# meteofrance/py4cast

Hardware: AMD Instinct MI355X
Metric: AR-training samples/sec (512x512x60 grid, 3-step rollout) (higher is better)
Workload: dtype bf16; 1 GPU; HalfUNet scaled_ar rollout T=3, grid 512x512x60 (+5 forcings, 4 statics), WeightedLoss(MSE), AdamW, B=2/GPU; global_batch=2, parallelism=dp1, border_size=0, setup_steps=2, accumulate_grad_batches=1, hip_graph=False, deterministic_library_solvers=False, full=False

## Files before the change

include/py4cast_hip.h:

```cpp
#ifndef PY4CAST_HIP_H
#define PY4CAST_HIP_H

#include <stddef.h>
#include <stdint.h>

#ifdef __cplusplus
extern "C" {
#endif

#define P4C_VERSION 100

typedef void* p4c_stream_t;

enum p4c_error {
    P4C_OK = 0,
    P4C_ERR_INVALID = -1,
    P4C_ERR_LAUNCH = -2,
    P4C_ERR_RUNTIME = -3,
    P4C_ERR_UNSUPPORTED = -4
};

enum p4c_dtype { P4C_F32 = 0, P4C_BF16 = 1 };

enum p4c_loss_kind { P4C_LOSS_MSE = 0, P4C_LOSS_L1 = 1 };
// ... 140 lines not shown
                 int B, int H, int W, int m_blocks, p4c_stream_t stream);

size_t p4c_conv_wgrad_workspace_bytes(int CI_pad, int ks);
int p4c_conv_stat_tiles(int compute, int storage, int CI, int B, int H, int W);
int p4c_conv_stat_tiles_ks(int compute, int storage, int CI, int ks, int B, int H, int W);
int p4c_conv_kernel_kind(int compute, int storage, int CI, int ks, int B, int H, int W);
int p4c_conv_wgrad(const void* in, int compute, int storage, int CI_pad, int ks, const float* in_scale, const float* in_shift,
                   int in_relu, const void* dout, int CO, int CI, float* grad, void* workspace, int B, int H, int W,
                   p4c_stream_t stream);
int p4c_conv_wgrad_nb(const void* in, const float* in_scale, const float* in_shift, int in_relu, const void* dA, const void* y,
                      const float* gamma, const float* nscale, const float* nshift, const float* rstd, const float* mean,
                      const float* k1, const float* k2, int CO, int CI, float* grad, void* workspace, int B, int H, int W,
                      p4c_stream_t stream);
int p4c_upsample_sum_bwd_x(int storage, const void* dS, int B, int H, int W, void* tx1, void* tx2, void* tx3, void* tx4,
                           p4c_stream_t stream);

int p4c_out_conv_bwd_slots(int B, int64_t N);
size_t p4c_out_conv_bwd_workspace_bytes(int B, int64_t N);
int p4c_out_conv_bwd(const void* dy, const void* wprep_dgrad, const void* y, const float* scale, const float* shift, const float* mean,
                     const float* rstd, void* dA, float* stat_partial, int CO, float* grad_w, void* workspace, int B, int64_t N,
                     p4c_stream_t stream);
int p4c_conv_wgrad_kernel_kind(int storage, int B, int H, int W);
int p4c_conv_compact_supported(int in_c, int out_c, int ks, int B, int H, int W);
int p4c_conv_fwd_compact(const void* in, int in_c, const void* wprep, int ks, void* out, int out_c, int B, int H, int W,
                         p4c_stream_t stream);
int p4c_conv_wgrad_compact(const void* in, int in_c, int ks, const void* dout, int dout_c, int CO, int CI, float* grad, void* workspace,
                           int B, int H, int W, p4c_stream_t stream);

typedef struct p4c_halfunet_desc {
    int32_t B, H, W;
    int32_t cin;
    int32_t cin_pad;
    int32_t cout;
    int32_t dx_channels;
    int32_t dtype;
    int32_t norm;
    int32_t groups;
    int32_t has_bias;
    float eps;
    float momentum;
    int32_t compute;
    int32_t weights_prepared;
    int32_t skip_out_conv;
} p4c_halfunet_desc;

int p4c_first_conv_tail_slots(int B, int H, int W);
int p4c_first_conv_tail(const void* x, int x_cs, int cin, const float* w, void* y, float* stat_partial, int B, int H, int W, p4c_stream_t stream);

int p4c_set_side_stream(p4c_stream_t side, void* const* events, int n_events);
int p4c_side_stream_defer(int on);
int p4c_side_stream_enable(int on);
long long p4c_side_stream_launch_count(void);
int p4c_side_stream_join(p4c_stream_t stream);
int p4c_graph_replace_memsets(void* graph, int* replaced, int* left);

int64_t p4c_halfunet_param_count(const p4c_halfunet_desc* d);
int p4c_halfunet_workspace_bytes(const p4c_halfunet_desc* d, size_t* saved_bytes, size_t* scratch_bytes);
int p4c_halfunet_prepare_weights(const p4c_halfunet_desc* d, const float* params, void* scratch, p4c_stream_t stream);
int p4c_halfunet_forward(const p4c_halfunet_desc* d, const void* x, const float* params, float* running, void* y,
                         void* saved, void* scratch, int training, p4c_stream_t stream);
int p4c_halfunet_tail(const p4c_halfunet_desc* d, const float* params, void* saved, const void** a, const float** a_scale,
                      const float** a_shift, const float** wout);
int p4c_halfunet_backward(const p4c_halfunet_desc* d, const void* x, const float* params, const void* dy, void* dx,
                          float* grads, void* saved, void* scratch, int training, p4c_stream_t stream);


enum p4c_activation { P4C_ACT_NONE = 0, P4C_ACT_RELU = 1, P4C_ACT_SILU = 2 };

int p4c_edge_gather_add_fwd(const void* base, const void* a, const int32_t* ia, const void* b, const int32_t* ib,
                            void* out, int64_t E, int C, int dtype, int act, p4c_stream_t stream);
int p4c_edge_gather_add_bwd(const void* dh, const void* base, const void* a, const int32_t* ia, const void* b,
                            const int32_t* ib, void* dpre, int64_t E, int C, int dtype, int act, p4c_stream_t stream);
int p4c_segment_sum(const void* msg, const int32_t* offsets, const int32_t* perm, const void* init, void* out,
                    int64_t N, int64_t E, int C, int dtype, int out_dtype, p4c_stream_t stream);
int p4c_segment_sum_pair(const void* msg, const int32_t* offsets_a, const int32_t* perm_a, void* out_a, int64_t Na,
                         const int32_t* offsets_b, const int32_t* perm_b, void* out_b, int64_t Nb, int64_t E, int C, int dtype,
                         p4c_stream_t stream);


int p4c_window_attn_fwd(const void* qkv, const float* bias_t, void* out, int B, int Hp, int Wp, int heads, int head_dim,
                        int ws, int shift, float scale, int dtype, p4c_stream_t stream);
size_t p4c_window_attn_bwd_workspace_bytes(int B, int Hp, int Wp, int heads, int ws);
int p4c_window_attn_bwd(const void* qkv, const float* bias_t, const void* dout, void* dqkv, float* dbias_t, void* workspace,
                        int B, int Hp, int Wp, int heads, int head_dim, int ws, int shift, float scale, int dtype,
                        p4c_stream_t stream);


int p4c_row_layernorm_fwd(const void* x, const void* res, const float* gamma, const float* beta, float eps, void* out,
                          int64_t R, int C, int dtype, p4c_stream_t stream);
size_t p4c_row_layernorm_bwd_workspace_bytes(int64_t R, int C, int dtype);
int p4c_row_layernorm_bwd(const void* dy, const void* x, const float* gamma, float eps, void* dx, float* dgamma, float* dbeta,
                          void* workspace, int64_t R, int C, int dtype, p4c_stream_t stream);
int p4c_row_layernorm_fwd_masked(const void* x, const void* res, const float* gamma, const float* beta, float eps, void* out, int64_t R,
                                 int C, int dtype, int Hp, int Wp, int H, int W, p4c_stream_t stream);
int p4c_row_layernorm_bwd_masked(const void* dy, const void* x, const float* gamma, float eps, void* dx, float* dgamma, float* dbeta,
                                 void* workspace, int64_t R, int C, int dtype, int Hp, int Wp, int H, int W, p4c_stream_t stream);
int p4c_row_add_layernorm_fwd(const void* x, const void* add, int64_t add_rows, const float* gamma, const float* beta, float eps,
                              void* sum_out, void* out, int64_t R, int C, int dtype, p4c_stream_t stream);
size_t p4c_row_add_layernorm_bwd_workspace_bytes(int64_t R, int C);
int p4c_row_add_layernorm_bwd(const void* dy, const void* t, const void* extra, const float* gamma, float eps, void* dt, float* dgamma,
                              float* dbeta, void* workspace, int64_t R, int C, int dtype, p4c_stream_t stream);
int p4c_sum_leading(const void* x, int dtype, int nb, int64_t n, float* out, int accumulate, p4c_stream_t stream);
size_t p4c_row_linear_wgrad_workspace_bytes(int64_t R, int K);
int p4c_row_linear_wgrad(const void* dy, const void* x, float* dw_db, void* workspace, int64_t R, int O, int K, int dtype,
                         p4c_stream_t stream);

// ... 197 lines not shown
```

py4cast_amd/_lib_model.py:

```python

import ctypes
from ctypes import c_float, c_int, c_int32, c_int64, c_size_t, c_void_p

P, I, L, F = c_void_p, c_int, c_int64, c_float


class HalfUNetDesc(ctypes.Structure):

    _fields_ = [
        ("B", c_int32), ("H", c_int32), ("W", c_int32),
        ("cin", c_int32), ("cin_pad", c_int32), ("cout", c_int32), ("dx_channels", c_int32),
        ("dtype", c_int32), ("norm", c_int32), ("groups", c_int32), ("has_bias", c_int32),
        ("eps", c_float), ("momentum", c_float), ("compute", c_int32),
        ("weights_prepared", c_int32), ("skip_out_conv", c_int32),
    ]


DP = ctypes.POINTER(HalfUNetDesc)


class RowMlpDesc(ctypes.Structure):

    _fields_ = [
        ("rows", c_int64), ("x", c_void_p), ("k", c_int32), ("k_real", c_int32), ("w1", c_void_p), ("ldw1", c_int32),
# ... 68 lines not shown
    "p4c_gemm_nt": [P, L, P, I, I, I, I, I, I, I, I, P, P, L, I, P, P, L, P, L, P, P, P],
    "p4c_gemm_tn": [P, L, P, L, I, I, I, I, I, I, I, P, P, I, I, P, P],
    "p4c_bnorm_finalize": [P, I, ctypes.c_double, I, P, P, F, F, P, P, P, P, P, P, P, P],
    "p4c_upconv_prep_weight": [P, I, I, P, P, P],
    "p4c_gemm_upconv_fwd": [P, L, P, P, I, I, I, I, I, P, L, P, P],
    "p4c_gemm_upconv_dgrad": [P, L, P, I, I, I, I, I, P, L, P, P],
    "p4c_gemm_upconv_wgrad": [P, L, P, L, I, I, I, I, I, P, P, I, P, P],
    "p4c_unet_enc_tail_fwd": [P, P, P, P, L, P, I, I, I, I, I, P],
    "p4c_unet_enc_tail_bwd": [P, P, L, P, L, P, P, P, P, P, I, I, I, I, I, P],
    "p4c_seg_patch_gather": [P, P, I, I, I, I, I, I, I, P],
    "p4c_seg_patch_scatter": [P, P, I, I, I, I, I, I, I, I, P],
    "p4c_seg_chan_ln_fwd": [P, P, P, F, P, P, L, I, P],
    "p4c_seg_chan_ln_bwd": [P, P, P, P, F, P, P, P, L, I, P],
    "p4c_seg_reduce_partials": [P, I, I, P, I, P, I, P],
    "p4c_seg_dw3x3_fwd": [P, P, P, P, I, I, I, I, P],
    "p4c_seg_dw3x3_dgrad": [P, P, P, I, I, I, I, P],
    "p4c_seg_dw3x3_wgrad": [P, P, P, I, I, I, I, P],
    "p4c_seg_sra_fwd": [P, P, P, P, I, I, I, I, F, P],
    "p4c_seg_sra_bwd": [P, P, P, P, P, P, P, P, I, I, I, I, F, P],
    "p4c_seg_upsum_fwd": [P, P, P, P, P, I, I, I, I, P],
    "p4c_seg_upsum_bwd": [P, P, P, P, I, I, I, I, P],
    "p4c_upsample_bilinear_ac_fwd": [P, P, I, I, I, I, I, P],
    "p4c_upsample_bilinear_ac_bwd": [P, P, I, I, I, I, I, P],
    "p4c_deeplab_stem_fwd": [P, P, P, P, P, I, I, I, I, P],
    "p4c_deeplab_stem_bwd": [P, P, P, P, P, P, P, P, P, I, I, I, I, P],
    "p4c_deeplab_colsum": [P, L, P, I, I, I, I, P],
    "p4c_deeplab_pool_head_fwd": [P, I, I, P, P, P, F, F, P, P, P, I, I, I, I, P, P, P, P, P],
    "p4c_deeplab_pool_head_bwd": [P, I, P, P, P, P, P, P, I, I, I, I, P, P, P, P, P, P],
    "p4c_deeplab_pool_broadcast": [P, P, I, I, I, P],
    "p4c_deeplab_assemble_fwd": [P, P, P, P, P, P, I, I, I, P],
    "p4c_deeplab_assemble_bwd": [P, P, P, P, P, I, I, I, P],
}
OTHER = {
    "p4c_conv_wgrad_workspace_bytes": ([I, I], c_size_t),
    "p4c_out_conv_bwd_slots": ([I, L], c_int),
    "p4c_first_conv_tail_slots": ([I, I, I], c_int),
    "p4c_out_conv_bwd_workspace_bytes": ([I, L], c_size_t),
    "p4c_conv_stat_tiles": ([I, I, I, I, I, I], c_int),
    "p4c_conv_stat_tiles_ks": ([I, I, I, I, I, I, I], c_int),
    "p4c_conv_kernel_kind": ([I, I, I, I, I, I, I], c_int),
    "p4c_conv_compact_supported": ([I, I, I, I, I, I], c_int),
    "p4c_halfunet_param_count": ([DP], c_int64),
    "p4c_window_attn_bwd_workspace_bytes": ([I, I, I, I, I], c_size_t),
    "p4c_row_layernorm_bwd_workspace_bytes": ([L, I, I], c_size_t),
    "p4c_row_linear_wgrad_workspace_bytes": ([L, I], c_size_t),
    "p4c_row_gemm_supported": ([I, I], c_int),
    "p4c_row_gemm_wgrad_supported": ([I, I, I], c_int),
    "p4c_row_gemm_wgrad_workspace_bytes": ([L, I, I, I], c_size_t),
    "p4c_row_mlp_bwd_workspace_bytes": ([L, I], c_size_t),
    "p4c_row_mlp_prepared_bytes": ([I], c_size_t),
    "p4c_node_proj_wgrad_workspace_bytes": ([L, I], c_size_t),
    "p4c_grad_reduce_pending": ([], c_int),
    "p4c_side_stream_launch_count": ([], ctypes.c_longlong),
    "p4c_row_add_layernorm_bwd_workspace_bytes": ([L, I], c_size_t),
    "p4c_gemm_nt_workspace_bytes": ([I, I, I], c_size_t),
    "p4c_gemm_nt_stat_blocks": ([I, I, I], c_int),
    "p4c_gemm_tn_workspace_bytes": ([I, I, I], c_size_t),
    "p4c_unet_enc_tail_bwd_blocks": ([I, I, I, I], c_int),
    "p4c_seg_chan_ln_bwd_blocks": ([L], c_int),
    "p4c_seg_dw3x3_wgrad_rows": ([I, I, I], c_int),
    "p4c_seg_sra_bwd_workspace_bytes": ([I, I, I, I], c_size_t),
    "p4c_deeplab_stem_bwd_blocks": ([I, I, I, I], c_int),
}
```

py4cast_amd/csrc/halfunet.cpp:

```cpp
#include <stdlib.h>

#include <atomic>
#include <functional>
#include <vector>

#include "kernels.hpp"

namespace p4c {
namespace {

constexpr int NF = 64;
constexpr int NLEV = 5;
constexpr int NCONV = 12;
constexpr int NWSLOT = 2 * NCONV + 3;

struct Layout {
    int esz;
    int64_t n[NLEV];
    int Hk[NLEV], Wk[NLEV];
    int64_t w[NCONV], gamma[NCONV], beta[NCONV], wout, nparams;
    int64_t Y[NCONV], P[NLEV], S, act_elems, norm_base, norm[NCONV], saved_bytes;
    int64_t wslot_floats;
    int64_t wprep, statp, wgradp[NCONV + 1], ocbp[2], nbwdp, k1i[2][NCONV], k2i[2][NCONV], tickets, f_floats, g_base, G0, G1, G2, TB, DY[2][NCONV], scratch_bytes;
    int G;
};

inline int conv_level(int i) { return i < 10 ? i / 2 : 0; }
inline int conv_cin(const p4c_halfunet_desc& d, int i) { return i == 0 ? d.cin : NF; }
inline int conv_cin_pad(const p4c_halfunet_desc& d, int i) { return i == 0 ? d.cin_pad : NF; }
inline int64_t align256(int64_t v) { return (v + 255) / 256 * 256; }
inline int dx_blocks(const p4c_halfunet_desc& d) { return d.dx_channels > 64 ? (d.dx_channels + 63) / 64 : 1; }

inline int stat_tiles(int compute, int storage, int CI, int B, int H, int W, int ks = 3) {
    if (compute == P4C_BF16) return conv_bf16_stat_slots(CI, storage, B, H, W, ks);
    return ((H + CONV_TH - 1) / CONV_TH) * ((W + CONV_TW - 1) / CONV_TW);
}

inline int prep_w(int compute, const float* w, int CO, int CI, int ks, int tf, int M_pad, int K_pad, void* out, hipStream_t st) {
    return compute == P4C_BF16 ? prep_weights_bf16(w, CO, CI, ks, tf, M_pad, K_pad, out, st)
                               : prep_weights(w, CO, CI, ks, tf, M_pad, K_pad, (float*)out, st);
}
inline int conv_fwd(int compute, int storage, const void* in, int CI, const void* wp, int ks, const float* sc, const float* sh,
                    int relu, void* out, int out_cs, float* statp, int B, int H, int W, int mblocks, hipStream_t st,
                    const BatchFin* fin = nullptr, const RingBwdStats* bst = nullptr, int* nblk_out = nullptr,
                    const NormBwdCoef* nb = nullptr) {
    return compute == P4C_BF16
               ? conv_fwd_bf16(in, storage, CI, wp, ks, sc, sh, relu, out, out_cs, statp, B, H, W, mblocks, st, fin, bst, nblk_out, nb)
               : conv_fwd_f32((const float*)in, CI, (const float*)wp, ks, sc, sh, relu, nullptr, (float*)out, out_cs, statp, B, H, W,
                              mblocks, st);
}
inline int conv_wgrad(int compute, int storage, const void* in, int CI, int ks, const float* sc, const float* sh, int relu,
                      const void* dout, float* partial, int G, int B, int H, int W, int CO, int CIreal, float* grad,
                      hipStream_t st, const NormBwdCoef* nb = nullptr) {
    return compute == P4C_BF16
               ? conv_wgrad_bf16(in, storage, CI, ks, sc, sh, relu, dout, partial, G, B, H, W, CO, CIreal, grad, st, nb)
               : conv_wgrad_f32((const float*)in, CI, ks, sc, sh, relu, (const float*)dout, partial, G, B, H, W, CO, CIreal, grad, st);
}

int check_desc(const p4c_halfunet_desc* d) {
    P4C_CHECK_ARG(d, "halfunet: null descriptor");
    P4C_CHECK_ARG(d->B > 0 && d->H > 0 && d->W > 0, "halfunet: bad shape");
    P4C_CHECK_ARG(d->H % 16 == 0 && d->W % 16 == 0, "halfunet: H and W must be multiples of 16 (got %dx%d)", d->H, d->W);
    P4C_CHECK_ARG(d->cin_pad > 0 && d->cin_pad <= 256 && d->cin_pad % 32 == 0,
                  "halfunet: cin_pad must be a multiple of 32 up to 256 (got %d)", d->cin_pad);
    P4C_CHECK_ARG(d->cin > 0 && d->cin <= d->cin_pad, "halfunet: cin out of range");
    P4C_CHECK_ARG(d->cout > 0 && d->cout <= 64, "halfunet: cout must be in 1..64 (got %d)", d->cout);
    P4C_CHECK_ARG(d->dx_channels >= 0 && d->dx_channels <= d->cin, "halfunet: bad dx_channels (%d, cin %d)", d->dx_channels, d->cin);
    P4C_CHECK_ARG(d->norm == 0 || (d->norm == 1 && d->groups > 0 && 64 % d->groups == 0), "halfunet: bad norm/groups");
    P4C_CHECK_ARG(d->compute == P4C_F32 || d->compute == P4C_BF16, "halfunet: compute must be P4C_F32 or P4C_BF16");
    P4C_CHECK_ARG(d->dtype == P4C_F32 || d->dtype == P4C_BF16, "halfunet: dtype must be P4C_F32 or P4C_BF16");
    if (d->dtype == P4C_BF16 && d->compute != P4C_BF16)
        return fail(P4C_ERR_UNSUPPORTED, "halfunet: bf16 activation storage needs compute = P4C_BF16");
    if (d->has_bias) return fail(P4C_ERR_UNSUPPORTED, "halfunet: conv bias (settings.bias=True) is not implemented");
    return P4C_OK;
}

void make_layout(const p4c_halfunet_desc& d, Layout& L) {
    L.esz = d.dtype == P4C_BF16 ? 2 : 4;
    for (int k = 0; k < NLEV; ++k) {
        L.Hk[k] = d.H >> k;
        L.Wk[k] = d.W >> k;
        L.n[k] = (int64_t)d.B * L.Hk[k] * L.Wk[k];
    }
    int64_t off = 0;
    for (int i = 0; i < NCONV; ++i) {
        L.w[i] = off; off += (int64_t)NF * conv_cin(d, i) * 9;
        L.gamma[i] = off; off += NF;
        L.beta[i] = off; off += NF;
    }
    L.wout = off; off += (int64_t)d.cout * NF;
    L.nparams = off;

    off = 0;
    for (int i = 0; i < NCONV; ++i) { L.Y[i] = off; off += L.n[conv_level(i)] * NF; }
    L.P[0] = -1;
    for (int k = 1; k < NLEV; ++k) { L.P[k] = off; off += L.n[k] * NF; }
    L.S = off; off += L.n[0] * NF;
    L.act_elems = off;
    L.norm_base = align256(off * L.esz);
    off = 0;
    for (int i = 0; i < NCONV; ++i) { L.norm[i] = off; off += 4 * (int64_t)d.B * NF; }
    L.saved_bytes = L.norm_base + off * (int64_t)sizeof(float);

    L.G = d.compute == P4C_BF16 ? num_cus() / 2 : num_cus();
    if (const char* e = diag_env("P4C_WGRAD_G")) { const int g = atoi(e); if (g > 0 && g <= num_cus()) L.G = g; }
    off = 0;
    {
        int64_t m = 96;
        if (d.cin_pad > m) m = d.cin_pad;
        if (64 * ((d.cin + 63) / 64) > m) m = 64 * ((d.cin + 63) / 64);
        L.wslot_floats = 9 * 64 * m;
    }
    L.wprep = off; off += (int64_t)NWSLOT * L.wslot_floats;
    const int64_t tps = conv_tiles_per_sample(d.H, d.W);
    {
        int64_t slots = tps > 4 * (int64_t)num_cus() ? tps : 4 * (int64_t)num_cus();
        for (int k = 0; k < NLEV; ++k) {
            const int64_t s = d.compute == P4C_BF16 ? conv_bf16_stat_slots(NF, d.dtype, d.B, L.Hk[k], L.Wk[k], 3) : 0;
            if (s > slots) slots = s;
        }
        const int64_t s0 = stat_tiles(d.compute, d.dtype, d.cin_pad, d.B, d.H, d.W);
        if (s0 > slots) slots = s0;
        if (first_conv_split_ok(d.compute, d.dtype, d.cin, d.cin_pad, d.B, d.H, d.W)) {
            const int64_t st = first_conv_tail_slots(d.B, d.H, d.W);
            if (st > slots) slots = st;
        }
        L.statp = off; off += (int64_t)d.B * slots * 128;
    }
    for (int i = 0; i <= NCONV; ++i) {
        const int lev = i < NCONV ? conv_level(i) : 0;
        int64_t tiles = (int64_t)d.B * conv_tiles_per_sample(L.Hk[lev], L.Wk[lev]);
        const int g = tiles < L.G ? (int)tiles : L.G;
        L.wgradp[i] = off; off += wgrad_partial_floats(i < NCONV ? conv_cin_pad(d, i) : NF, i < NCONV ? 3 : 1, g);
    }
    for (int s = 0; s < 2; ++s) {
        L.ocbp[s] = off;
        if (d.dtype == P4C_BF16) off += (int64_t)d.B * out_conv_bwd_slots(d.B, (int64_t)d.H * d.W) * 4096;
    }
    L.nbwdp = off; off += (int64_t)d.B * NORM_BWD_MAX_BLOCKS * 128;
    for (int s = 0; s < 2; ++s)
        for (int i = 0; i < NCONV; ++i) {
            L.k1i[s][i] = off; off += (int64_t)d.B * NF;
            L.k2i[s][i] = off; off += (int64_t)d.B * NF;
        }
    L.tickets = off; off += 64;
    L.f_floats = off;
    L.g_base = align256(off * (int64_t)sizeof(float));
    off = 0;
    L.G0 = off; off += L.n[0] * NF;
    L.G1 = off; off += L.n[0] * NF;
    L.G2 = off; off += L.n[0] * NF;
    L.TB = off; off += L.n[0] * NF;
    for (int s = 0; s < 2; ++s)
        for (int i = 0; i < NCONV; ++i) { L.DY[s][i] = off; off += L.n[conv_level(i)] * NF; }
    L.scratch_bytes = L.g_base + off * L.esz;
}

struct WS {
    const Layout& L;
    char* saved;
    char* scratch;
    void* act(int64_t elem_off) const { return saved + elem_off * L.esz; }
    float* nrm(int64_t float_off) const { return reinterpret_cast<float*>(saved + L.norm_base) + float_off; }
    float* f(int64_t float_off) const { return reinterpret_cast<float*>(scratch) + float_off; }
    void* g(int64_t elem_off) const { return scratch + L.g_base + elem_off * L.esz; }
};

struct Norm { float *scale, *shift, *mean, *rstd; };
inline Norm norm_at(const WS& ws, int i, int B) {
    float* p = ws.nrm(ws.L.norm[i]);
    return {p, p + (int64_t)B * NF, p + 2 * (int64_t)B * NF, p + 3 * (int64_t)B * NF};
}

inline void* wslot(const WS& ws, int slot) { return ws.f(ws.L.wprep + (int64_t)slot * ws.L.wslot_floats); }

int prepare_weights(const p4c_halfunet_desc& d, const WS& ws, const float* params, int which, hipStream_t st) {
    const Layout& L = ws.L;
    PrepBatch pb;
    pb.n = 0;
    pb.bf16 = d.compute == P4C_BF16;
    for (int i = 0; i < NCONV; ++i) {
        if (which & 1) pb.job[pb.n++] = {params + L.w[i], wslot(ws, i), NF, conv_cin(d, i), 9, 0, 64, conv_cin_pad(d, i)};
        if (which & 2) pb.job[pb.n++] = {params + L.w[i], wslot(ws, NCONV + i), NF, conv_cin(d, i), 9, 1, i == 0 ? 64 * dx_blocks(d) : 64, NF};
    }
    if (which & 1) pb.job[pb.n++] = {params + L.wout, wslot(ws, 2 * NCONV), d.cout, NF, 1, 0, 64, NF};
// ... 1 lines not shown
        pb.job[pb.n++] = {params + L.w[0], wslot(ws, 2 * NCONV + 2), NF, d.cin, 9, 0, 64, NF};
    if (which & 2) pb.job[pb.n++] = {params + L.wout, wslot(ws, 2 * NCONV + 1), d.cout, NF, 1, 1, 64, NF};
    pb.zero_words = reinterpret_cast<unsigned int*>(ws.f(L.tickets));
    pb.n_zero = 64;
    return prep_weights_batch(pb, st);
}

int conv_block_fwd(const p4c_halfunet_desc& d, const WS& ws, int i, const void* in, const Norm* in_norm, const float* params,
                   float* running, int training, hipStream_t st) {
    const Layout& L = ws.L;
    const int lev = conv_level(i), H = L.Hk[lev], W = L.Wk[lev];
    void* wp = wslot(ws, i);
    const bool batch_stats = (d.norm == 1) || training;
    float* statp = batch_stats ? ws.f(L.statp) : nullptr;
    Norm nm = norm_at(ws, i, d.B);
    float* rm = running ? running + (int64_t)i * 128 : nullptr;
    float* rv = running ? rm + 64 : nullptr;
    const char* ie = diag_env("P4C_NO_INKERNEL_FINALIZE");
    const bool no_infin = ie && ie[0] == '1';
    const char* ia = diag_env("P4C_INKERNEL_FINALIZE_ALL");
    const bool all_levels = ia && ia[0] == '1';
    const bool infin = batch_stats && d.norm == 0 && d.compute == P4C_BF16 && !no_infin && (all_levels || lev > 0) &&
                       conv_bf16_is_ring(d.dtype, conv_cin_pad(d, i), 3, 1, NF, d.B, H, W);
    BatchFin fin{};
    if (infin) {
        fin = BatchFin{statp, reinterpret_cast<unsigned int*>(ws.f(L.tickets)), params + L.gamma[i], params + L.beta[i], rm, rv,
                       nm.scale, nm.shift, nm.mean, nm.rstd, (double)d.B * H * W, d.eps, d.momentum, d.B};
    }
    int ntiles = stat_tiles(d.compute, d.dtype, conv_cin_pad(d, i), d.B, H, W);
    if (i == 0 && !in_norm && first_conv_split_ok(d.compute, d.dtype, d.cin, d.cin_pad, d.B, H, W)) {
        P4C_TRY(launch_conv_bf16_rows_wide_pixels(in, d.cin_pad, wslot(ws, 2 * NCONV + 2), ws.act(L.Y[i]), d.B, H, W, st));
        P4C_TRY(launch_first_conv_tail(in, d.cin_pad, d.cin, params + L.w[0], ws.act(L.Y[i]), statp, d.B, H, W, st));
        ntiles = first_conv_tail_slots(d.B, H, W);
    } else {
        P4C_TRY(conv_fwd(d.compute, d.dtype, in, conv_cin_pad(d, i), wp, 3, in_norm ? in_norm->scale : nullptr,
                         in_norm ? in_norm->shift : nullptr, in_norm ? 1 : 0, ws.act(L.Y[i]), NF, statp, d.B, H, W, 1, st,
                         infin ? &fin : nullptr));
    }
    if (infin) return P4C_OK;
    if (batch_stats) {
        P4C_TRY(norm_finalize(statp, ntiles, d.B, (int64_t)H * W, d.norm,
                              d.groups, params + L.gamma[i], params + L.beta[i], d.eps, d.momentum,
                              d.norm == 0 ? rm : nullptr, d.norm == 0 ? rv : nullptr, nm.scale, nm.shift, nm.mean, nm.rstd, st));
    } else {
        P4C_CHECK_ARG(running, "halfunet: eval-mode BatchNorm needs the running statistics");
        P4C_TRY(norm_eval(d.B, params + L.gamma[i], params + L.beta[i], d.eps, rm, rv, nm.scale, nm.shift, nm.mean,
                          nm.rstd, st));
    }
    return P4C_OK;
}

constexpr unsigned kOrderFlags = hipEventDisableTiming | hipEventDisableSystemFence;
void count_side_launches(long long n);
struct SideStream {
    hipStream_t stream = nullptr;
    std::vector<hipEvent_t> events;
    size_t next = 0;
    bool enabled = true;
    bool external = false;
    std::vector<std::function<int(hipStream_t)>> pending;
    int every = 2;
    bool defer = false;
    unsigned long long calls = 0;
    hipEvent_t set_done[2] = {nullptr, nullptr};
    bool set_recorded[2] = {false, false};
    hipEvent_t dy_read = nullptr;
    int own_events() {
        if (dy_read) return P4C_OK;
        for (int i = 0; i < 2; ++i) P4C_CHECK_HIP(hipEventCreateWithFlags(&set_done[i], kOrderFlags));
        P4C_CHECK_HIP(hipEventCreateWithFlags(&dy_read, kOrderFlags));
        return P4C_OK;
    }
    int init() {
        if (stream || external) return P4C_OK;
        const char* e = diag_env("P4C_SIDE_STREAM");
        enabled = !(e && e[0] == '0');
        if (const char* n = diag_env("P4C_SIDE_EVERY")) { const int v = atoi(n); if (v > 0) every = v; }
        if (!enabled) return P4C_OK;
        const char* pr = diag_env("P4C_SIDE_PRIO");
        if (pr && pr[0] != '0') {
            int lo = 0, hi = 0;
            P4C_CHECK_HIP(hipDeviceGetStreamPriorityRange(&lo, &hi));
            P4C_CHECK_HIP(hipStreamCreateWithPriority(&stream, hipStreamNonBlocking, atoi(pr) < 0 ? lo : hi));
        } else {
            P4C_CHECK_HIP(hipStreamCreateWithFlags(&stream, hipStreamNonBlocking));
        }
        return P4C_OK;
    }
    int flush(hipStream_t from) {
        if (pending.empty()) return P4C_OK;
        P4C_TRY(order(from, stream));
        count_side_launches((long long)pending.size());
        for (auto& job : pending) P4C_TRY(job(stream));
        pending.clear();
        return P4C_OK;
    }
    int event(hipEvent_t* ev) {
        if (next == events.size()) {
            if (external)
                return fail(P4C_ERR_INVALID, "p4c_halfunet_backward: the caller's %zu ordering events are used up "
                                             "(p4c_set_side_stream: pass at least 8)", events.size());
            hipEvent_t e;
            P4C_CHECK_HIP(hipEventCreateWithFlags(&e, kOrderFlags));
            events.push_back(e);
        }
        *ev = events[next++];
        return P4C_OK;
    }
    int order(hipStream_t from, hipStream_t to) {
        hipEvent_t ev;
        P4C_TRY(event(&ev));
        P4C_CHECK_HIP(hipEventRecord(ev, from));
        P4C_CHECK_HIP(hipStreamWaitEvent(to, ev, 0));
        return P4C_OK;
    }
};
thread_local SideStream g_side;
std::atomic<int> g_side_enable_request{-1};
std::atomic<long long> g_side_launches{0};
void count_side_launches(long long n) { g_side_launches.fetch_add(n); }
int apply_side_request() {
    const int req = g_side_enable_request.load();
    if (req < 0 || g_side.external) return P4C_OK;
    if (req && !g_side.stream) P4C_CHECK_HIP(hipStreamCreateWithFlags(&g_side.stream, hipStreamNonBlocking));
    g_side.enabled = req != 0;
    return P4C_OK;
}

inline void* block_grad(const WS& ws, int i) { return ws.g(ws.L.DY[g_side.calls & 1][i]); }

inline unsigned int* bwd_ticket(const p4c_halfunet_desc& d, const WS& ws) {
    return (d.norm == 0 && d.dtype == P4C_BF16) ? reinterpret_cast<unsigned int*>(ws.f(ws.L.tickets)) + 1 : nullptr;
}
inline BwdFin bwd_fin(const p4c_halfunet_desc& d, const WS& ws, int i, const float* params, float* grads, int training) {
    const Layout& L = ws.L;
    const int lev = conv_level(i);
    return BwdFin{bwd_ticket(d, ws), params + L.gamma[i], grads + L.gamma[i], grads + L.beta[i], ws.f(L.k1i[g_side.calls & 1][i]),
                  ws.f(L.k2i[g_side.calls & 1][i]), (float)d.B * (float)((int64_t)L.Hk[lev] * L.Wk[lev]), d.B,
                  ((d.norm == 1) || training) ? 1 : 0};
}

int conv_block_bwd(const p4c_halfunet_desc& d, const WS& ws, int i, const void* in, const Norm* in_norm, void* din,
                   const float* params, float* grads, int training, hipStream_t st, int pre_nblk = 0, int* next_nblk = nullptr,
                   bool pre_finalized = false) {
    const Layout& L = ws.L;
    const int lev = conv_level(i), H = L.Hk[lev], W = L.Wk[lev];
    Norm nm = norm_at(ws, i, d.B);
    const int stats_training = (d.norm == 1) || training;
    void* g = block_grad(ws, i);
    const int cip = conv_cin_pad(d, i);
    const bool dgrad_takes_pass1 = din && in_norm && i > 0;
    static const bool nb_all = [] { const char* e = diag_env("P4C_NB_ALL"); return !(e && e[0] == '0'); }();
    const bool nbf = (!dgrad_takes_pass1 || nb_all) && d.compute == P4C_BF16 && conv_bf16_norm_bwd_fused_ok(d.dtype, NF, d.B, H, W) &&
                     (i > 0 || dx_blocks(d) == 1) &&
                     (cip == NF || (cip <= 96 && nb_all && diag_env("P4C_NO_NB0") == nullptr && conv_wgrad_bf16_takes_nb(d.dtype, cip, 3, d.B)));
    P4C_TRY(norm_bwd(d.dtype, g, ws.act(L.Y[i]), nm.scale, nm.shift, nm.mean, nm.rstd, params + L.gamma[i], 1, d.B,
                     (int64_t)H * W, d.norm, d.groups, stats_training, ws.f(L.nbwdp), ws.f(L.k1i[g_side.calls & 1][i]), ws.f(L.k2i[g_side.calls & 1][i]),
                     grads + L.gamma[i], grads + L.beta[i], nbf ? nullptr : g, st, pre_nblk, bwd_ticket(d, ws), pre_finalized));
    const NormBwdCoef nb{ws.act(L.Y[i]), params + L.gamma[i], nm.scale, nm.shift, nm.rstd, nm.mean,
                         ws.f(L.k1i[g_side.calls & 1][i]), ws.f(L.k2i[g_side.calls & 1][i])};
    int64_t ntiles = (int64_t)d.B * conv_tiles_per_sample(H, W);
    const int G = ntiles < L.G ? (int)ntiles : L.G;
    const int compute = d.compute, dtype = d.dtype, Bn = d.B, cin = conv_cin(d, i);
    const float* isc = in_norm ? in_norm->scale : nullptr;
    const float* ish = in_norm ? in_norm->shift : nullptr;
    const int irelu = in_norm ? 1 : 0;
    float* wpart = ws.f(L.wgradp[i]);
    float* gw = grads + L.w[i];
    auto job = [=](hipStream_t s) {
        return conv_wgrad(compute, dtype, in, cip, 3, isc, ish, irelu, g, wpart, G, Bn, H, W, NF, cin, gw, s, nbf ? &nb : nullptr);
    };
    if (g_side.enabled) {
        g_side.pending.push_back(job);
        const char* f1 = diag_env("P4C_FLUSH_AT_1");
        const bool at1 = i == 1 && !g_side.external && !(f1 && f1[0] == '0');
        if ((int)g_side.pending.size() >= g_side.every || at1) P4C_TRY(g_side.flush(st));
    } else {
        P4C_TRY(job(st));
    }
    if (next_nblk) *next_nblk = 0;
    if (din) {
        const char* fe = diag_env("P4C_NO_FUSED_REDUCE");
        const bool fuse_off = fe && fe[0] == '1';
        const char* nbe = diag_env("P4C_NB_BST");
        const bool nb_bst = nbe && nbe[0] == '1';
        const bool fuse = !fuse_off && next_nblk && in_norm && i > 0 && d.compute == P4C_BF16 && (!(nbf && dgrad_takes_pass1) || nb_bst) &&
                          conv_bf16_bwd_stats_ok(d.dtype, d.B, H, W);
        const RingBwdStats bst{in, in_norm ? in_norm->scale : nullptr, in_norm ? in_norm->shift : nullptr,
                               in_norm ? in_norm->mean : nullptr, in_norm ? in_norm->rstd : nullptr};
        const int nblk = i == 0 ? dx_blocks(d) : 1;
        if (nblk == 1) {
            P4C_TRY(conv_fwd(d.compute, d.dtype, g, NF, wslot(ws, NCONV + i), 3, nullptr, nullptr, 0, din, 64, fuse ? ws.f(L.nbwdp) : nullptr,
                             d.B, H, W, 1, st, nullptr, fuse ? &bst : nullptr, fuse ? next_nblk : nullptr, nbf ? &nb : nullptr));
        } else if (d.compute == P4C_BF16 && conv_bf16_is_rows(d.dtype, NF, 3, 1, 64 * nblk, d.B, H, W)) {
            const int64_t wblk = (int64_t)9 * 64 * 64 * (d.compute == P4C_BF16 ? 2 : 4);
            for (int m = 0; m < nblk; ++m)
                P4C_TRY(conv_fwd(d.compute, d.dtype, g, NF, (char*)wslot(ws, NCONV + i) + m * wblk, 3, nullptr, nullptr, 0,
                                 (char*)din + (int64_t)m * 64 * L.esz, 64 * nblk, nullptr, d.B, H, W, 1, st));
        } else {
            P4C_TRY(conv_fwd(d.compute, d.dtype, g, NF, wslot(ws, NCONV + i), 3, nullptr, nullptr, 0, din, 64 * nblk, nullptr, d.B, H, W,
                             nblk, st));
        }
    }
    return P4C_OK;
}

}
}

using namespace p4c;

extern "C" int p4c_set_side_stream(p4c_stream_t side, void* const* events, int n_events) {
    SideStream& sd = g_side;
    if (!side) {
        if (sd.external) { sd.stream = nullptr; sd.events.clear(); sd.external = false; sd.enabled = true; }
        return P4C_OK;
    }
    P4C_CHECK_ARG(events && n_events >= 8, "p4c_set_side_stream: needs >= 8 ordering events (hipEvent_t, timing disabled)");
    sd.stream = as_stream(side);
    sd.events.assign(reinterpret_cast<hipEvent_t const*>(events), reinterpret_cast<hipEvent_t const*>(events) + n_events);
    sd.next = 0;
    sd.external = true;
    sd.enabled = true;
    return P4C_OK;
}
// ... 45 lines not shown
            P4C_TRY(pool_fwd(d.dtype, ws.act(L.Y[2 * k + 1]), n2.scale, n2.shift, d.B, L.Hk[k], L.Wk[k], ws.act(L.P[k + 1]), st));
        }
    }
    {
        const void* ys[NLEV];
        const float *sc[NLEV], *sh[NLEV];
        for (int k = 0; k < NLEV; ++k) {
            Norm n2 = norm_at(ws, 2 * k + 1, d.B);
            ys[k] = ws.act(L.Y[2 * k + 1]); sc[k] = n2.scale; sh[k] = n2.shift;
        }
        P4C_TRY(upsum_fwd(d.dtype, ys, sc, sh, d.B, d.H, d.W, ws.act(L.S), st));
    }
    P4C_TRY(conv_block_fwd(d, ws, 10, ws.act(L.S), nullptr, params, running, training, st));
    Norm nd1 = norm_at(ws, 10, d.B);
    P4C_TRY(conv_block_fwd(d, ws, 11, ws.act(L.Y[10]), &nd1, params, running, training, st));
    Norm nd2 = norm_at(ws, 11, d.B);
    if (d.skip_out_conv) return P4C_OK;
    P4C_TRY(conv_fwd(d.compute, d.dtype, ws.act(L.Y[11]), NF, wslot(ws, 2 * NCONV), 1, nd2.scale, nd2.shift, 1, y, NF, nullptr, d.B, d.H, d.W, 1, st));
    return P4C_OK;
}

extern "C" int p4c_halfunet_tail(const p4c_halfunet_desc* dp, const float* params, void* savedv, const void** a, const float** a_scale,
                                 const float** a_shift, const float** wout) {
    P4C_TRY(check_desc(dp));
    P4C_CHECK_ARG(params && savedv && a && a_scale && a_shift && wout, "p4c_halfunet_tail: null pointer");
    Layout L;
    make_layout(*dp, L);
    const WS ws{L, (char*)savedv, nullptr};
    const Norm n = norm_at(ws, 11, dp->B);
    *a = ws.act(L.Y[11]);
    *a_scale = n.scale;
    *a_shift = n.shift;
    *wout = params + L.wout;
    return P4C_OK;
}

extern "C" int p4c_halfunet_backward(const p4c_halfunet_desc* dp, const void* x, const float* params, const void* dy,
                                     void* dx, float* grads, void* savedv, void* scratchv, int training,
                                     p4c_stream_t stream) {
    P4C_TRY(check_desc(dp));
    P4C_CHECK_ARG(x && params && dy && grads && savedv && scratchv, "p4c_halfunet_backward: null pointer");
    const p4c_halfunet_desc& d = *dp;
    P4C_CHECK_ARG(dx || d.dx_channels == 0, "p4c_halfunet_backward: dx is null but dx_channels > 0");
    Layout L;
    make_layout(d, L);
    hipStream_t st = as_stream(stream);
    const WS ws{L, (char*)savedv, (char*)scratchv};
    void *G0 = ws.g(L.G0), *G1 = ws.g(L.G1), *G2 = ws.g(L.G2), *TB = ws.g(L.TB);
    if (!d.weights_prepared) P4C_TRY(prepare_weights(d, ws, params, 2, st));
    P4C_TRY(g_side.init());
    P4C_TRY(apply_side_request());
    g_side.next = 0;
    g_side.pending.clear();
    hipStreamCaptureStatus cap = hipStreamCaptureStatusNone;
    if (hipStreamIsCapturing(st, &cap) != hipSuccess) { (void)hipGetLastError(); cap = hipStreamCaptureStatusNone; }
    const bool plain_stream = g_side.enabled && !g_side.external && cap == hipStreamCaptureStatusNone;
    const bool deferring = plain_stream && g_side.defer;
    if (plain_stream) {
        P4C_TRY(g_side.own_events());
        ++g_side.calls;
        const int set = (int)(g_side.calls & 1);
        if (g_side.set_recorded[set]) P4C_CHECK_HIP(hipStreamWaitEvent(st, g_side.set_done[set], 0));
    }
    struct BwdPhase { BwdPhase() { prof_set_backward(true); } ~BwdPhase() { prof_set_backward(false); } } bwd_phase;
    static const bool batch_reduce = [] { const char* e = diag_env("P4C_WGRAD_BATCH"); return !(e && e[0] == '0'); }();
    WgradCollect reduce_jobs;
    struct Collect {
        explicit Collect(WgradCollect* c) { wgrad_collect_into(c); }
        ~Collect() { wgrad_collect_into(nullptr); }
    } collect(batch_reduce ? &reduce_jobs : nullptr);

    Norm nd2 = norm_at(ws, 11, d.B);
    int pre11 = 0;
    const bool fused_out = d.compute == P4C_BF16 && out_conv_bwd_ok(d.dtype, d.B, (int64_t)d.H * d.W);
    if (fused_out) {
        float* wpart = ws.f(L.ocbp[g_side.calls & 1]);
        P4C_TRY(launch_out_conv_bwd(dy, wslot(ws, 2 * NCONV + 1), ws.act(L.Y[11]), nd2.scale, nd2.shift, nd2.mean, nd2.rstd,
                                    block_grad(ws, 11), ws.f(L.nbwdp), wpart, d.B, (int64_t)d.H * d.W, st, &pre11));
        P4C_TRY(wgrad_reduce(wpart, d.B * pre11, 1, NF, 0, NF, d.cout, NF, grads + L.wout, st));
    } else {
        int64_t ntiles = (int64_t)d.B * conv_tiles_per_sample(d.H, d.W);
        const int G = ntiles < L.G ? (int)ntiles : L.G;
        hipStream_t wst = st;
        if (g_side.enabled) {
            P4C_TRY(g_side.order(st, g_side.stream));
            wst = g_side.stream;
            count_side_launches(1);
        }
        P4C_TRY(conv_wgrad(d.compute, d.dtype, ws.act(L.Y[11]), NF, 1, nd2.scale, nd2.shift, 1, dy, ws.f(L.wgradp[NCONV]), G, d.B, d.H,
                           d.W, d.cout, NF, grads + L.wout, wst));
        if (deferring) P4C_CHECK_HIP(hipEventRecord(g_side.dy_read, g_side.stream));
        const char* fe = diag_env("P4C_NO_FUSED_REDUCE");
        const bool fuse11 = !(fe && fe[0] == '1') && d.compute == P4C_BF16 && conv_bf16_is_rows(d.dtype, NF, 1, 1, NF, d.B, d.H, d.W) &&
                            conv_bf16_bwd_stats_ok(d.dtype, d.B, d.H, d.W);
        if (fuse11) {
            const RingBwdStats bst{ws.act(L.Y[11]), nd2.scale, nd2.shift, nd2.mean, nd2.rstd};
            P4C_TRY(conv_fwd(d.compute, d.dtype, dy, NF, wslot(ws, 2 * NCONV + 1), 1, nullptr, nullptr, 0, block_grad(ws, 11), NF,
                             ws.f(L.nbwdp), d.B, d.H, d.W, 1, st, nullptr, &bst, &pre11));
        } else {
            P4C_TRY(conv_fwd(d.compute, d.dtype, dy, NF, wslot(ws, 2 * NCONV + 1), 1, nullptr, nullptr, 0, block_grad(ws, 11), NF, nullptr,
                             d.B, d.H, d.W, 1, st));
        }
    }
    Norm nd1 = norm_at(ws, 10, d.B);
    int nxt = 0;
    P4C_TRY(conv_block_bwd(d, ws, 11, ws.act(L.Y[10]), &nd1, block_grad(ws, 10), params, grads, training, st, pre11, &nxt));
    P4C_TRY(conv_block_bwd(d, ws, 10, ws.act(L.S), nullptr, G0, params, grads, training, st, nxt));

    void* tx[4];
    {
        int64_t off = 0;
        for (int k = 1; k < NLEV; ++k) { tx[k - 1] = (char*)TB + off * L.esz; off += L.n[0] * NF >> k; }
        P4C_TRY(up_bwd_x4(d.dtype, G0, d.B, d.H, d.W, tx, st));
    }
    void *a = G1, *b = G2;
    for (int k = NLEV - 1; k >= 0; --k) {
        const int Hk = L.Hk[k], Wk = L.Wk[k];
        Norm n2 = norm_at(ws, 2 * k + 1, d.B);
        Norm n1 = norm_at(ws, 2 * k, d.B);
        const void* dP = (k + 1 < NLEV) ? a : nullptr;
        const char* fe = diag_env("P4C_NO_FUSED_REDUCE");
        const bool fuse_off = fe && fe[0] == '1';
        const bool fuse = !fuse_off && d.dtype == P4C_BF16;
        int pre = 0;
        bool finished = false;
        float* part = fuse ? ws.f(L.nbwdp) : nullptr;
        const BwdFin fin = bwd_fin(d, ws, 2 * k + 1, params, grads, training);
        if (k > 0) {
            P4C_TRY(enc_out_bwd(d.dtype, tx[k - 1], d.H, 1 << k, nullptr, dP, ws.act(L.Y[2 * k + 1]), n2.scale, n2.shift, d.B, Hk, Wk,
                                block_grad(ws, 2 * k + 1), st, n2.mean, n2.rstd, part, &pre, &fin, &finished));
        } else {
            P4C_TRY(enc_out_bwd(d.dtype, nullptr, d.H, 1, G0, dP, ws.act(L.Y[1]), n2.scale, n2.shift, d.B, Hk, Wk, block_grad(ws, 1), st,
                                n2.mean, n2.rstd, part, &pre, &fin, &finished));
        }
        int nxt1 = 0;
        P4C_TRY(conv_block_bwd(d, ws, 2 * k + 1, ws.act(L.Y[2 * k]), &n1, block_grad(ws, 2 * k), params, grads, training, st, pre, &nxt1,
                               finished));
        if (k > 0) {
            P4C_TRY(conv_block_bwd(d, ws, 2 * k, ws.act(L.P[k]), nullptr, b, params, grads, training, st, nxt1));
            void* t = a; a = b; b = t;
        } else {
            P4C_TRY(conv_block_bwd(d, ws, 0, x, nullptr, d.dx_channels > 0 ? dx : nullptr, params, grads, training, st, nxt1));
        }
    }
    if (g_side.enabled) {
        if (g_side.pending.empty()) P4C_TRY(g_side.order(st, g_side.stream));
        P4C_TRY(g_side.flush(st));
        P4C_TRY(wgrad_reduce_batch(reduce_jobs, g_side.stream));
        if (plain_stream) {
            const int set = (int)(g_side.calls & 1);
            P4C_CHECK_HIP(hipEventRecord(g_side.set_done[set], g_side.stream));
            g_side.set_recorded[set] = true;
        }
        if (deferring) {
            if (!fused_out) P4C_CHECK_HIP(hipStreamWaitEvent(st, g_side.dy_read, 0));
        } else
            P4C_TRY(g_side.order(g_side.stream, st));
    } else {
        P4C_TRY(wgrad_reduce_batch(reduce_jobs, st));
    }
    return P4C_OK;
}

extern "C" int p4c_side_stream_enable(int on) {
    g_side_enable_request.store(on != 0 ? 1 : 0);
    P4C_TRY(g_side.init());
    return apply_side_request();
}

extern "C" long long p4c_side_stream_launch_count(void) { return g_side_launches.load(); }

extern "C" int p4c_side_stream_defer(int on) {
    g_side.defer = on != 0;
    return P4C_OK;
}

extern "C" int p4c_side_stream_join(p4c_stream_t stream) {
    SideStream& sd = g_side;
    if (!sd.enabled || !sd.stream || sd.external) return P4C_OK;
    hipStreamCaptureStatus cap = hipStreamCaptureStatusNone;
    if (hipStreamIsCapturing(as_stream(stream), &cap) != hipSuccess) { (void)hipGetLastError(); cap = hipStreamCaptureStatusNone; }
    if (cap != hipStreamCaptureStatusNone) return P4C_OK;
    sd.next = 0;
    return sd.order(sd.stream, as_stream(stream));
}

extern "C" int p4c_prep_weights(const float* w, int CO, int CI, int ks, int transpose_flip, int M_pad, int K_pad,
                                void* out, int compute, p4c_stream_t stream) {
    P4C_CHECK_ARG(w && out, "p4c_prep_weights: null pointer");
    P4C_CHECK_ARG((ks == 1 || ks == 3) && M_pad % 64 == 0 && K_pad % 32 == 0, "p4c_prep_weights: bad ks / padding");
    P4C_CHECK_ARG(compute == P4C_F32 || compute == P4C_BF16, "p4c_prep_weights: bad compute type");
    return prep_w(compute, w, CO, CI, ks, transpose_flip, M_pad, K_pad, out, as_stream(stream));
}

extern "C" int p4c_conv_stat_tiles(int compute, int storage, int CI, int B, int H, int W) {
    return stat_tiles(compute, storage, CI, B, H, W);
}

extern "C" int p4c_conv_stat_tiles_ks(int compute, int storage, int CI, int ks, int B, int H, int W) {
    return stat_tiles(compute, storage, CI, B, H, W, ks);
}

extern "C" int p4c_conv_kernel_kind(int compute, int storage, int CI, int ks, int B, int H, int W) {
    if (compute != P4C_BF16) return 0;
    if (conv_bf16_is_rows(storage, CI, ks, 1, 64, B, H, W)) return 2;
    return conv_bf16_is_ring(storage, CI, ks, 1, 64, B, H, W) ? 1 : 0;
}

extern "C" int p4c_conv_fwd(const void* in, int compute, int storage, int CI, const void* wprep, int ks,
                            const float* in_scale, const float* in_shift, int in_relu, const float* bias, void* out,
                            int out_cs, float* stat_partial, int B, int H, int W, int m_blocks, p4c_stream_t stream) {
    P4C_CHECK_ARG(in && wprep && out, "p4c_conv_fwd: null pointer");
    P4C_CHECK_ARG((in_scale == nullptr) == (in_shift == nullptr), "p4c_conv_fwd: scale and shift go together");
    P4C_CHECK_ARG(m_blocks >= 1 && out_cs >= 64 * m_blocks && out_cs % 4 == 0, "p4c_conv_fwd: bad out_cs / m_blocks");
    P4C_CHECK_ARG(!stat_partial || m_blocks == 1, "p4c_conv_fwd: statistics need m_blocks == 1");
    P4C_CHECK_ARG(compute == P4C_F32 || compute == P4C_BF16, "p4c_conv_fwd: bad compute type %d", compute);
    P4C_CHECK_ARG(storage == P4C_F32 || (storage == P4C_BF16 && compute == P4C_BF16), "p4c_conv_fwd: bad storage type");
    if (compute == P4C_BF16 && bias) return fail(P4C_ERR_UNSUPPORTED, "p4c_conv_fwd: bias is not implemented for P4C_BF16");
    if (compute == P4C_BF16)
        return conv_fwd_bf16(in, storage, CI, wprep, ks, in_scale, in_shift, in_relu, out, out_cs, stat_partial, B, H, W,
                             m_blocks, as_stream(stream));
    return conv_fwd_f32((const float*)in, CI, (const float*)wprep, ks, in_scale, in_shift, in_relu, bias, (float*)out, out_cs,
                        stat_partial, B, H, W, m_blocks, as_stream(stream));
}

extern "C" size_t p4c_conv_wgrad_workspace_bytes(int CI_pad, int ks) {
    return (size_t)wgrad_partial_floats(CI_pad, ks, num_cus()) * sizeof(float);
}

extern "C" int p4c_conv_wgrad(const void* in, int compute, int storage, int CI_pad, int ks, const float* in_scale,
                              const float* in_shift, int in_relu, const void* dout, int CO, int CI, float* grad,
                              void* workspace, int B, int H, int W, p4c_stream_t stream) {
    P4C_CHECK_ARG(in && dout && grad && workspace, "p4c_conv_wgrad: null pointer");
    P4C_CHECK_ARG(CO <= 64 && CI <= CI_pad, "p4c_conv_wgrad: CO must be <= 64 and CI <= CI_pad");
    P4C_CHECK_ARG(compute == P4C_F32 || compute == P4C_BF16, "p4c_conv_wgrad: bad compute type");
    P4C_CHECK_ARG(storage == P4C_F32 || (storage == P4C_BF16 && compute == P4C_BF16), "p4c_conv_wgrad: bad storage type");
    int64_t ntiles = (int64_t)B * conv_tiles_per_sample(H, W);
    const int G = ntiles < num_cus() ? (int)ntiles : num_cus();
// ... 71 lines not shown
```

Measured before the change: 437.6 samples/s.

## Carry deferred weight-gradient jobs across backward calls to overlap with next step

In deferred side-stream mode, level-0 wgrad jobs are held and later launched on the side stream, and at the end of backward the remaining wgrad jobs plus their reduction are carried into the next backward call instead of being flushed immediately. The carried jobs run once the next call's output-conv backward has finished, so weight-gradient work overlaps with the next rollout step's dgrad chain rather than serialising at the end. A separate grid size knob for level-0 wgrad is added, and join/capture paths drain carried work. This adds state across calls and a risk of stale gradients if the join is not called before the optimizer reads them.

```diff
diff --git a/include/py4cast_hip.h b/include/py4cast_hip.h
--- a/include/py4cast_hip.h
+++ b/include/py4cast_hip.h
@@ -216,6 +216,7 @@
 int p4c_side_stream_enable(int on);
 long long p4c_side_stream_launch_count(void);
 int p4c_side_stream_join(p4c_stream_t stream);
+long long p4c_side_stream_carried_count(void);
 int p4c_graph_replace_memsets(void* graph, int* replaced, int* left);
 
 int64_t p4c_halfunet_param_count(const p4c_halfunet_desc* d);
diff --git a/py4cast_amd/_lib_model.py b/py4cast_amd/_lib_model.py
--- a/py4cast_amd/_lib_model.py
+++ b/py4cast_amd/_lib_model.py
@@ -144,6 +144,7 @@
     "p4c_node_proj_wgrad_workspace_bytes": ([L, I], c_size_t),
     "p4c_grad_reduce_pending": ([], c_int),
     "p4c_side_stream_launch_count": ([], ctypes.c_longlong),
+    "p4c_side_stream_carried_count": ([], ctypes.c_longlong),
     "p4c_row_add_layernorm_bwd_workspace_bytes": ([L, I], c_size_t),
     "p4c_gemm_nt_workspace_bytes": ([I, I, I], c_size_t),
     "p4c_gemm_nt_stat_blocks": ([I, I, I], c_int),
diff --git a/py4cast_amd/csrc/halfunet.cpp b/py4cast_amd/csrc/halfunet.cpp
--- a/py4cast_amd/csrc/halfunet.cpp
+++ b/py4cast_amd/csrc/halfunet.cpp
@@ -23,6 +23,7 @@
     int64_t wslot_floats;
     int64_t wprep, statp, wgradp[NCONV + 1], ocbp[2], nbwdp, k1i[2][NCONV], k2i[2][NCONV], tickets, f_floats, g_base, G0, G1, G2, TB, DY[2][NCONV], scratch_bytes;
     int G;
+    int Gw;
 };
 
 inline int conv_level(int i) { return i < 10 ? i / 2 : 0; }
@@ -104,6 +105,8 @@
 
     L.G = d.compute == P4C_BF16 ? num_cus() / 2 : num_cus();
     if (const char* e = diag_env("P4C_WGRAD_G")) { const int g = atoi(e); if (g > 0 && g <= num_cus()) L.G = g; }
+    L.Gw = L.G;
+    if (const char* e = diag_env("P4C_WGRAD_WINDOW_G")) { const int g = atoi(e); if (g > 0 && g <= num_cus()) L.Gw = g; }
     off = 0;
     {
         int64_t m = 96;
@@ -130,7 +133,8 @@
     for (int i = 0; i <= NCONV; ++i) {
         const int lev = i < NCONV ? conv_level(i) : 0;
         int64_t tiles = (int64_t)d.B * conv_tiles_per_sample(L.Hk[lev], L.Wk[lev]);
-        const int g = tiles < L.G ? (int)tiles : L.G;
+        const int gmax = lev == 0 && L.Gw > L.G ? L.Gw : L.G;
+        const int g = tiles < gmax ? (int)tiles : gmax;
         L.wgradp[i] = off; off += wgrad_partial_floats(i < NCONV ? conv_cin_pad(d, i) : NF, i < NCONV ? 3 : 1, g);
     }
     for (int s = 0; s < 2; ++s) {
@@ -238,13 +242,22 @@
 
 constexpr unsigned kOrderFlags = hipEventDisableTiming | hipEventDisableSystemFence;
 void count_side_launches(long long n);
+void count_side_carried(long long n);
 struct SideStream {
     hipStream_t stream = nullptr;
     std::vector<hipEvent_t> events;
     size_t next = 0;
     bool enabled = true;
     bool external = false;
-    std::vector<std::function<int(hipStream_t)>> pending;
+    using Job = std::function<int(hipStream_t)>;
+    std::vector<Job> pending;
+    bool hold = false;
+    std::vector<Job> held;
+    std::vector<Job> carried;
+    WgradCollect carried_reduce;
+    bool carried_batch = false;
+    bool carried_any = false;
+    int carried_set = 0;
     int every = 2;
     bool defer = false;
     unsigned long long calls = 0;
@@ -281,6 +294,33 @@
         pending.clear();
         return P4C_OK;
     }
+    int run_carried(WgradCollect* current) {
+        if (!carried_any) return P4C_OK;
+        wgrad_collect_into(carried_batch ? &carried_reduce : nullptr);
+        count_side_launches((long long)carried.size());
+        int rc = P4C_OK;
+        for (auto& job : carried)
+            if ((rc = job(stream)) != P4C_OK) break;
+        wgrad_collect_into(current);
+        count_side_carried(-(long long)carried.size());
+        carried.clear();
+        carried_any = false;
+        if (rc == P4C_OK) rc = wgrad_reduce_batch(carried_reduce, stream);
+        carried_reduce.n = 0;
+        P4C_TRY(rc);
+        P4C_CHECK_HIP(hipEventRecord(set_done[carried_set], stream));
+        set_recorded[carried_set] = true;
+        return P4C_OK;
+    }
+    int open_window(hipStream_t from, WgradCollect* current) {
+        if (!carried_any && held.empty()) return P4C_OK;
+        P4C_TRY(order(from, stream));
+        P4C_TRY(run_carried(current));
+        count_side_launches((long long)held.size());
+        for (auto& job : held) P4C_TRY(job(stream));
+        held.clear();
+        return P4C_OK;
+    }
     int event(hipEvent_t* ev) {
         if (next == events.size()) {
             if (external)
@@ -305,6 +345,8 @@
 std::atomic<int> g_side_enable_request{-1};
 std::atomic<long long> g_side_launches{0};
 void count_side_launches(long long n) { g_side_launches.fetch_add(n); }
+std::atomic<long long> g_side_carried{0};
+void count_side_carried(long long n) { g_side_carried.fetch_add(n); }
 int apply_side_request() {
     const int req = g_side_enable_request.load();
     if (req < 0 || g_side.external) return P4C_OK;
@@ -346,7 +388,8 @@
     const NormBwdCoef nb{ws.act(L.Y[i]), params + L.gamma[i], nm.scale, nm.shift, nm.rstd, nm.mean,
                          ws.f(L.k1i[g_side.calls & 1][i]), ws.f(L.k2i[g_side.calls & 1][i])};
     int64_t ntiles = (int64_t)d.B * conv_tiles_per_sample(H, W);
-    const int G = ntiles < L.G ? (int)ntiles : L.G;
+    const int Gl = lev == 0 && g_side.hold ? L.Gw : L.G;
+    const int G = ntiles < Gl ? (int)ntiles : Gl;
     const int compute = d.compute, dtype = d.dtype, Bn = d.B, cin = conv_cin(d, i);
     const float* isc = in_norm ? in_norm->scale : nullptr;
     const float* ish = in_norm ? in_norm->shift : nullptr;
@@ -356,7 +399,9 @@
     auto job = [=](hipStream_t s) {
         return conv_wgrad(compute, dtype, in, cip, 3, isc, ish, irelu, g, wpart, G, Bn, H, W, NF, cin, gw, s, nbf ? &nb : nullptr);
     };
-    if (g_side.enabled) {
+    if (g_side.enabled && g_side.hold && lev == 0) {
+        g_side.held.push_back(job);
+    } else if (g_side.enabled) {
         g_side.pending.push_back(job);
         const char* f1 = diag_env("P4C_FLUSH_AT_1");
         const bool at1 = i == 1 && !g_side.external && !(f1 && f1[0] == '0');
@@ -508,10 +553,21 @@
     P4C_TRY(apply_side_request());
     g_side.next = 0;
     g_side.pending.clear();
+    g_side.held.clear();
     hipStreamCaptureStatus cap = hipStreamCaptureStatusNone;
     if (hipStreamIsCapturing(st, &cap) != hipSuccess) { (void)hipGetLastError(); cap = hipStreamCaptureStatusNone; }
     const bool plain_stream = g_side.enabled && !g_side.external && cap == hipStreamCaptureStatusNone;
     const bool deferring = plain_stream && g_side.defer;
+    const char* he = diag_env("P4C_WGRAD_HOLD");
+    const char* ce = diag_env("P4C_WGRAD_CARRY");
+    g_side.hold = deferring && !(he && he[0] == '0');
+    if (g_side.carried_any && !deferring) {
+        if (cap != hipStreamCaptureStatusNone)
+            return fail(P4C_ERR_INVALID, "p4c_halfunet_backward: weight gradients of a deferred call are outstanding at the start of a "
+                                         "stream capture (p4c_side_stream_join first)");
+        P4C_TRY(g_side.order(st, g_side.stream));
+        P4C_TRY(g_side.run_carried(nullptr));
+    }
     if (plain_stream) {
         P4C_TRY(g_side.own_events());
         ++g_side.calls;
@@ -529,6 +585,11 @@
     Norm nd2 = norm_at(ws, 11, d.B);
     int pre11 = 0;
     const bool fused_out = d.compute == P4C_BF16 && out_conv_bwd_ok(d.dtype, d.B, (int64_t)d.H * d.W);
+    const bool carry = deferring && fused_out && !(ce && ce[0] == '0');
+    if (g_side.carried_any && !carry) {
+        P4C_TRY(g_side.order(st, g_side.stream));
+        P4C_TRY(g_side.run_carried(batch_reduce ? &reduce_jobs : nullptr));
+    }
     if (fused_out) {
         float* wpart = ws.f(L.ocbp[g_side.calls & 1]);
         P4C_TRY(launch_out_conv_bwd(dy, wslot(ws, 2 * NCONV + 1), ws.act(L.Y[11]), nd2.scale, nd2.shift, nd2.mean, nd2.rstd,
@@ -569,6 +630,7 @@
         for (int k = 1; k < NLEV; ++k) { tx[k - 1] = (char*)TB + off * L.esz; off += L.n[0] * NF >> k; }
         P4C_TRY(up_bwd_x4(d.dtype, G0, d.B, d.H, d.W, tx, st));
     }
+    if (g_side.enabled) P4C_TRY(g_side.open_window(st, batch_reduce ? &reduce_jobs : nullptr));
     void *a = G1, *b = G2;
     for (int k = NLEV - 1; k >= 0; --k) {
         const int Hk = L.Hk[k], Wk = L.Wk[k];
@@ -599,7 +661,19 @@
             P4C_TRY(conv_block_bwd(d, ws, 0, x, nullptr, d.dx_channels > 0 ? dx : nullptr, params, grads, training, st, nxt1));
         }
     }
-    if (g_side.enabled) {
+    if (g_side.enabled && carry) {
+        g_side.carried = std::move(g_side.held);
+        for (auto& job : g_side.pending) g_side.carried.push_back(std::move(job));
+        g_side.held.clear();
+        g_side.pending.clear();
+        count_side_carried((long long)g_side.carried.size());
+        g_side.carried_reduce = reduce_jobs;
+        g_side.carried_batch = batch_reduce;
+        g_side.carried_set = (int)(g_side.calls & 1);
+        g_side.carried_any = true;
+    } else if (g_side.enabled) {
+        for (auto& job : g_side.held) g_side.pending.push_back(std::move(job));
+        g_side.held.clear();
         if (g_side.pending.empty()) P4C_TRY(g_side.order(st, g_side.stream));
         P4C_TRY(g_side.flush(st));
         P4C_TRY(wgrad_reduce_batch(reduce_jobs, g_side.stream));
@@ -633,13 +707,19 @@
 
 extern "C" int p4c_side_stream_join(p4c_stream_t stream) {
     SideStream& sd = g_side;
-    if (!sd.enabled || !sd.stream || sd.external) return P4C_OK;
+    if ((!sd.enabled && !sd.carried_any) || !sd.stream || sd.external) return P4C_OK;
     hipStreamCaptureStatus cap = hipStreamCaptureStatusNone;
     if (hipStreamIsCapturing(as_stream(stream), &cap) != hipSuccess) { (void)hipGetLastError(); cap = hipStreamCaptureStatusNone; }
     if (cap != hipStreamCaptureStatusNone) return P4C_OK;
     sd.next = 0;
+    if (sd.carried_any) {
+        P4C_TRY(sd.order(as_stream(stream), sd.stream));
+        P4C_TRY(sd.run_carried(nullptr));
+    }
     return sd.order(sd.stream, as_stream(stream));
 }
+
+extern "C" long long p4c_side_stream_carried_count(void) { return g_side_carried.load(); }
 
 extern "C" int p4c_prep_weights(const float* w, int CO, int CI, int ks, int transpose_flip, int M_pad, int K_pad,
                                 void* out, int compute, p4c_stream_t stream) {
```

Result: slower. 422.9 samples/s (-3.4%).
